# tensor4all/tensor4all-rs

Hardware: AMD Instinct MI355X
Metric: TCI2 full-sweep GF/s (d=30, chi=256 fp64) (higher is better)
Workload: dtype f64

## Files before the change

### tensor4all-rs_amd/csrc/kernels.hpp

```cpp
#pragma once

#include <hip/hip_runtime.h>

#include <cstddef>
#include <cstdint>

#include "../../include/t4a_testfunctions.h"

namespace t4a {

struct RrluWorkspace;

struct RrluPlan {
    int W = 1;
    int T = 256;
    int cpw = 0;
    int Mld = 0;
    size_t lds_bytes = 0;
};

RrluPlan rrlu_make_plan(int M, int N, int num_cus);

struct RrluArgs {
    const double* A;
// ... 90 lines not shown
    unsigned long long* trace;
    int fused;
    const uint64_t* rowacc;
    const uint64_t* colacc;
    FnDevice fn;
    unsigned done_token;
    const int* dims;
    int dims_swap;
    unsigned dev_token;
    const int* rowmap;
    int ts_u64;
};
bool rrlu_reg_make_plan(int M, int N, int num_cus, RrluRegPlan* out);
size_t rrlu_reg_keys_bytes(const RrluRegPlan& plan);
size_t rrlu_reg_cols_bytes(const RrluRegPlan& plan, int M);
void rrlu_reg_launch(const RrluRegPlan& plan, const RrluRegArgs& args, hipStream_t stream, bool keys_zeroed = false);

struct XcdSpecArgs {
    double* out;
    const uint64_t* dep_acc;
    const uint64_t* w_site;
    const uint64_t* ext_acc;
    const int* ext_cnt;
    const uint64_t* ind_acc;
    const int* ind_cnt;
    unsigned* tile_counter;
    int total, d;
    FnDevice fn;
};
struct RrluXcdPlan {
    int W = 1;
    int RPT = 1, CPT = 1;
    int grid = 8;
    size_t lds_bytes = 0;
    int wg = 0;
    int K = 1;
    bool big() const { return K > 1 || RPT > 16; }
};
struct RrluXcdArgs {
    const double* A;
    double* Aout;
    double* urows;
    int M, N;
    int max_steps;
    double rel_tol, abs_tol;
    int tie_row_major;
    int out_transposed;
    int W;
    int xcc;
    unsigned* ticket;
    unsigned ticket_base;
    int* row_perm;
    int* col_perm;
    int* iresult;
    double* dresult;
    double* pivot_vals;
    unsigned long long* keys;
    unsigned salt;
    double spec_frac;
    unsigned long long* stamps;
    unsigned long long* h_block;
    int block_u64;
    const int* dims;
    int dims_swap;
    const int* rowmap;
    XcdSpecArgs spec;
    int ts_u64;
};
bool rrlu_xcd_make_plan(int M, int N, RrluXcdPlan* out, bool any_size = false, int max_w = 32, bool allow_big = false);
size_t rrlu_xcd_keys_bytes(const RrluXcdPlan& plan);
size_t rrlu_xcd_cols_bytes(const RrluXcdPlan& plan, int M);
struct RrluXcdGroupArgs {
    RrluXcdArgs p[8];
};
void rrlu_xcd2_launch(const RrluXcdPlan& plan, const RrluXcdArgs& args, hipStream_t stream);
void rrlu_xcd2m_launch(const RrluXcdPlan& plan, const RrluXcdArgs& args, hipStream_t stream);
void rrlu_xcd2_group_launch(const RrluXcdPlan& plan, const RrluXcdGroupArgs& args, bool tie_row_major, hipStream_t stream);
bool rrlu_wg_make_plan(int M, int N, RrluXcdPlan* out, int spec_blocks = 0);
void rrlu_wg_launch(const RrluXcdPlan& plan, const RrluXcdArgs& args, hipStream_t stream);
void rrlu_wg_group_launch(const RrluXcdPlan& plan, const RrluXcdGroupArgs& args, bool tie_row_major, hipStream_t stream);
bool rrlu_w1_make_plan(int M, int N, RrluXcdPlan* out, int spec_blocks = 0);
void rrlu_w1_launch(const RrluXcdPlan& plan, const RrluXcdArgs& args, hipStream_t stream);
void rrlu_w1_group_launch(const RrluXcdPlan& plan, const RrluXcdGroupArgs& args, bool tie_row_major, hipStream_t stream);

void pi_eval_launch(const FnDevice& fn, const uint64_t* rowacc, int M, const uint64_t* colacc, int N, double* out,
                    int ld, bool transpose_out, unsigned long long* max_abs_bits, hipStream_t stream);
struct PiJob {
    const uint64_t* rowacc;
    const uint64_t* colacc;
    double* out;
    unsigned long long* max_abs_bits;
    int M, N, ld, pad_;
};
void pi_eval_batched_launch(const FnDevice& fn, const PiJob* d_jobs, int n_jobs, int max_M, int max_N, hipStream_t stream);
struct PackJob {
    const double* src;
    double* core;
    const int* info;
    int ld, L, S, R, last, pad_;
};
struct LuProblem;
constexpr int FILL_SMALL_MAX_N = 32, FILL_SMALL_MAX_RHS = 64;
void fill_small_launch(const FnDevice& fn, const PiJob* d_pis, const LuProblem* d_lups, const PackJob* d_packs, int n_jobs, int last_site,
                       hipStream_t stream);
void stage_copy_launch(const uint64_t* pinned_src, uint64_t* dst, size_t count, hipStream_t stream);
void absmax_launch(const double* data, size_t count, unsigned long long* max_abs_bits, hipStream_t stream);

constexpr int CHAIN_MAX_SET = 1024;
struct ChainTab {
    uint64_t* code;
    uint64_t* acc;
    int* cnt;
};
struct ChainCommon {
    ChainTab I, J, HI, HJ;
    ChainTab mI, mJ;
    int cap, K;
    const uint64_t* w;
    int total;
    const int* ldim;
    const int* woff;
    int forward, use_extras;
    int one_site;
    uint64_t* ind_code;
    uint64_t* ind_acc;
    int* ind_cnt;
    int ind_cap;
    uint64_t* dep_code;
    uint64_t* dep_acc;
    int dep_cap;
    int* rowmap;
    int* dims;
    int* hdims;
    uint64_t* snap_dst;
    int* snap_cnt_dst;
    size_t snap_words;
    int n_sites;
    uint64_t* zero_a;
    size_t zero_a_words;
    uint64_t* zero_b;
    size_t zero_b_words;
};
struct ChainPrepArgs {
    int b;
    int do_build;
    int with_rowmap;
    int prev_b;
    const int* prev_iresult;
    const int* prev_rowperm;
    const int* prev_colperm;
    unsigned prev_token;
    unsigned long long* dbg;
    int defer_host_writes;
};
struct ChainWalkArgs {
    char* blocks;
    size_t block_bytes, off_piv, off_rp, off_cp, off_ts;
    double* pi;
    int n_bonds;
    int max_steps;
    double rel_tol, abs_tol;
    double* factors;
    size_t factors_stride;
    unsigned token_base;
    int timed;
    int lean_prep;
    unsigned long long* phase_ticks;
};
void chain_walk_launch(const ChainCommon& c, const FnDevice& fn, const ChainWalkArgs& w, int columns, hipStream_t stream);
void chain_indep_launch(const ChainCommon& c, int n_bonds, hipStream_t stream);
void chain_last_core_launch(const ChainCommon& c, const FnDevice& fn, double* core, int max_entries, hipStream_t stream);
void chain_prep_launch(const ChainCommon& c, const ChainPrepArgs& a, hipStream_t stream);
void chain_pi_launch(const ChainCommon& c, const FnDevice& fn, int b, int n_dep_ub, int n_ind_ub, double* out, hipStream_t stream);

constexpr int CHAIN_GROUP_MAX = 8;
struct ChainGroupSlot {
    ChainCommon c;
    FnDevice fn;
    double* pi;
};
struct ChainPrepGroupArgs {
    ChainPrepArgs a[CHAIN_GROUP_MAX];
};
void chain_indep_group_launch(const ChainGroupSlot* d_slots, int n_handles, int n_bonds, hipStream_t stream);
void chain_prep_group_launch(const ChainGroupSlot* d_slots, const ChainPrepGroupArgs& a, int n_handles, hipStream_t stream);
void chain_pi_group_launch(const ChainGroupSlot* d_slots, int n_handles, int b, int n_dep_ub, int n_ind_ub, hipStream_t stream);

struct GemmDesc {
    int m, n, k;
    const double* A; int lda; long long strideA; int transA;
    const double* B; int ldb; long long strideB; int transB;
    double* C; int ldc; long long strideC;
    double alpha, beta;
    int batch;
    int ksplit = 1;
    double* partial = nullptr;
};
void gemm_launch(const GemmDesc& d, hipStream_t stream);

constexpr int LUCI_LEFT_CORES_MAX_JOBS = 80;
constexpr int LUCI_LEFT_CORES_MAX_RANK = 16;
struct LeftCoreJob {
    const double* lu;
    const int* dims;
    const int* iresult;
    const int* row_perm;
    double* core;
    int S;
    unsigned token;
};
struct LeftCoreJobs {
    LeftCoreJob j[LUCI_LEFT_CORES_MAX_JOBS];
};
void luci_left_cores_batched_launch(const LeftCoreJobs& jobs, int n_jobs, int max_rows, hipStream_t stream);
bool luci_factors_small_launch(const double* lu, int M, int N, int rk, const int* row_perm, const int* col_perm, bool left_orth,
                               double* left, double* right, hipStream_t stream);
void transpose_launch(const double* in, int rows, int cols, int ldi, double* out, int ldo, hipStream_t stream);

struct TrsmProblem {
    const double* T; int ldt; int n;
    double* B; int ldb; int nrhs;
    int lower; int unit_diag;
    const int* skip_flag;
};
void trsm_left_batched_launch(const TrsmProblem* d_problems, int n_problems, int max_n, int max_nrhs, hipStream_t stream);

struct LuProblem {
    double* A; int lda; int n;
    int* piv;
    int* info;
    double* B; int ldb; int nrhs;
    const unsigned long long* pmax_bits;
};
void lu_batched_launch(const LuProblem* d_problems, int n_problems, int max_n, hipStream_t stream);
constexpr int LU_MAX_PANEL_STEPS = 128;
bool lu_forward_blocked_launch(const LuProblem* d_problems, int n_problems, int max_n, int max_nrhs, hipStream_t stream, int avoid_xcc = -1,
                               unsigned* tickets = nullptr);
bool lu_solve_blocked_launch(const LuProblem* d_problems, int n_problems, int max_n, int max_nrhs, hipStream_t stream, int avoid_xcc = -1,
                             unsigned* tickets = nullptr);

void gather_launch(const double* in, int ldi, const int* rows, int nrows, const int* cols, int ncols, double* out,
                   int ldo, hipStream_t stream);
void scatter_rows_launch(const double* in, int ldi, const int* rows, int nrows, int ncols, double* out, int ldo,
                         hipStream_t stream);
void scatter_cols_launch(const double* in, int ldi, int nrows, const int* cols, int ncols, double* out, int ldo,
                         hipStream_t stream);
void fill_launch(double* p, size_t count, double value, hipStream_t stream);
void seq_matmul_launch(const double* A, int lda, const double* B, int ldb, double* C, int ldc, size_t M, size_t N, size_t K,
                       hipStream_t stream);
void set_identity_launch(double* p, int m, int n, int ld, hipStream_t stream);

struct TtCoreDesc { const double* data; int l, d, r; };
void tt_evaluate_launch(const TtCoreDesc* d_cores, int n_sites, int max_bond, const uint32_t* d_idx, int n_pts,
                        double* d_out, hipStream_t stream);


void core_reshape_launch(const double* in, int L, int S, int R, int mode, double* out, hipStream_t stream);
constexpr int PERMUTE_MAX_RANK = 16;
void permute_launch(const double* in, const size_t* dims, const size_t* perm, int rank, double* out, hipStream_t stream);
void tt_sum_launch(const TtCoreDesc* d_cores, int n_sites, int max_bond, double* d_out, hipStream_t stream);
void tt_norm2_step_launch(const TtCoreDesc& core, const double* d_cur, bool first, double* d_nxt, hipStream_t stream);
void tt_env_left_launch(const TtCoreDesc* d_cores, int split, int max_bond, const uint32_t* d_idx, int n_items,
                        double* d_out, int ld, hipStream_t stream);
void tt_env_right_launch(const TtCoreDesc* d_cores, int n_sites, int split, int max_bond, const uint32_t* d_idx,
                         int n_items, double* d_out, int ld, hipStream_t stream);
void tt_env_dot_launch(const double* d_left, const double* d_right, int len, int ld, const uint32_t* d_il,
                       const uint32_t* d_ir, size_t n_pts, double* d_out, hipStream_t stream);

struct MpoSiteJob {
    const double* A;
    const double* B;
    double* C;
    unsigned long long off;
    int la, s1, k, ra, lb, t, rb, pad_;
};
void mpo_site_contract_launch(const MpoSiteJob* d_jobs, int n_jobs, unsigned long long total, hipStream_t stream);

constexpr int SMALL_CAP = 16;
constexpr int SMALL_TILE = 32;
constexpr int SMALL_MAX_SITES = 32;
constexpr int SMALL_MAX_ITER = 64;
constexpr int SMALL_MAX_W = 512;
struct SmallHeader {
    int n, K, fid, total;
    int max_iter, ncheck, sweep_strategy, flags;
    int max_bond_dim, cap_in, tile_max, pad1;
    double tolerance, max_sample_value;
    double params[T4A_FN_MAX_PARAMS];
    int o_ldim, o_woff, o_w, o_cnt, o_code, o_acc, o_cores, bytes;
};
struct SmallOutHeader {
    int status;
    int iters_done;
    int converged, termination, n_pivot_errors, final_done, hist_valid, reason;
    double max_sample_value;
    unsigned long long clocks[12];
};
struct SmallOutLayout {
    size_t o_err, o_rank, o_bond, o_pe, o_shapes, o_cdims, o_cnt, o_code, o_hcnt, o_hcode, o_flag, bytes;
};
__host__ __device__ inline SmallOutLayout small_out_layout(int n)
{
    SmallOutLayout L;
    size_t o = (sizeof(SmallOutHeader) + 15) / 16 * 16;
    L.o_err = o;    o += sizeof(double) * SMALL_MAX_ITER;
    L.o_rank = o;   o += sizeof(int) * SMALL_MAX_ITER;
// ... 51 lines not shown
```

### tensor4all-rs_amd/csrc/kernels_chain.hip

```cpp
#include "kernels.hpp"
#include "kernels_rrlu_w1_body.hpp"

namespace t4a {

namespace {

__device__ __forceinline__ const char* chain_kernarg_base()
{
#if defined(__HIP_DEVICE_COMPILE__)
    return (const char*)__builtin_amdgcn_kernarg_segment_ptr();
#else
    return nullptr;
#endif
}

constexpr int CHAIN_T = 1024;
constexpr int WALK_T = 1024;
constexpr int CHAIN_HASH = 4096;

__device__ __forceinline__ unsigned chain_hash(unsigned long long c)
{
    c ^= c >> 33;
    c *= 0xff51afd7ed558ccdull;
    c ^= c >> 29;
// ... 135 lines not shown

constexpr int WALK_MAX_BONDS = 128;
constexpr int WALK_MAX_LIST = 64;
constexpr int WALK_MAX_IND = 32;
constexpr int WALK_MAX_W = 512;
struct WalkShared {
    int prev_ires[4];
    int perm_rp[WALK_MAX_LIST], perm_cp[WALK_MAX_LIST];
    int np;
    int pad_;
    uint64_t par_code[WALK_MAX_LIST], par_acc[WALK_MAX_LIST * T4A_FN_MAX_ACC];
    uint64_t dep_code[WALK_MAX_LIST], dep_acc[WALK_MAX_LIST * T4A_FN_MAX_ACC];
    int dims[WALK_MAX_BONDS * 4];
    int ind_cnt[WALK_MAX_BONDS];
    uint64_t ind_code[2][WALK_MAX_IND], ind_acc[2][WALK_MAX_IND * T4A_FN_MAX_ACC];
    uint64_t ext_code[2][WALK_MAX_LIST], ext_acc[2][WALK_MAX_LIST * T4A_FN_MAX_ACC];
    int ext_cnt[2];
    int ldim[WALK_MAX_BONDS + 1], woff[WALK_MAX_BONDS + 1];
    uint64_t w[WALK_MAX_W];
};

__device__ __forceinline__ void chain_prep_body(const ChainCommon& c, const ChainPrepArgs& p, unsigned long long* dbg = nullptr, WalkShared* ws = nullptr)
{
    unsigned long long dbg_last = dbg ? wall_clock64() : 0ull;
    auto stamp = [&](int slot) {
        if (dbg) {
            const unsigned long long now = wall_clock64();
            if (threadIdx.x == 0) dbg[slot] += now - dbg_last;
            dbg_last = now;
        }
    };
    __shared__ unsigned long long hkeys[CHAIN_HASH];
    __shared__ int wave_sums[CHAIN_T / 64];
    __shared__ int s_srcpos[CHAIN_MAX_SET];
    __shared__ int s_poison;
    const int tid = threadIdx.x;
    const int K = c.K;
    const size_t cap = (size_t)c.cap;
    if (tid == 0) s_poison = 0;
    __syncthreads();

    int n_prev_dep = 0;
    if (p.prev_b >= 0) {
        const int pb = p.prev_b;
        const int* pd = c.dims + (size_t)pb * 4;
        const int pm = pd[0], pn = pd[1];
        const bool bad = pd[2] != 0 || p.prev_iresult[1] != 0 || p.prev_iresult[3] != (int)p.prev_token || pm <= 0 || pn <= 0;
        if (bad) {
            if (tid == 0) s_poison = 1;
        } else {
            const int r = p.prev_iresult[0];
            const int cnt = r > 0 ? r : 1;
            if (cnt > c.cap || cnt > pm || cnt > pn) {
                if (tid == 0) s_poison = 1;
            } else {
                n_prev_dep = c.forward ? pm : pn;
                const uint64_t* const pind_code = ws ? ws->ind_code[pb & 1] : c.ind_code + (size_t)pb * c.ind_cap;
                const uint64_t* const pind_acc = ws ? ws->ind_acc[pb & 1] : c.ind_acc + (size_t)pb * c.ind_cap * K;
                const uint64_t* rcode = c.forward ? c.dep_code : pind_code;
                const uint64_t* racc = c.forward ? c.dep_acc : pind_acc;
                const uint64_t* ccode = c.forward ? pind_code : c.dep_code;
                const uint64_t* cacc = c.forward ? pind_acc : c.dep_acc;
                const size_t oi = (size_t)(pb + 1) * cap, oj = (size_t)pb * cap;
                for (int k = tid; k < cnt; k += (int)blockDim.x) {
                    const int ri = r > 0 ? p.prev_rowperm[k] : 0, ci = r > 0 ? p.prev_colperm[k] : 0;
                    const uint64_t rc = rcode[ri], cc = ccode[ci];
                    c.I.code[oi + k] = rc;
                    c.J.code[oj + k] = cc;
                    if (ws) ws->par_code[k] = c.forward ? rc : cc;
                    if (!p.defer_host_writes) {
                        c.mI.code[oi + k] = rc;
                        c.mJ.code[oj + k] = cc;
                    }
                    for (int q = 0; q < K; ++q) {
                        const uint64_t ra = racc[(size_t)ri * K + q], ca = cacc[(size_t)ci * K + q];
                        c.I.acc[(oi + k) * K + q] = ra;
                        c.J.acc[(oj + k) * K + q] = ca;
                        if (ws) ws->par_acc[(size_t)k * K + q] = c.forward ? ra : ca;
                        if (!p.defer_host_writes) {
                            c.mI.acc[(oi + k) * K + q] = ra;
                            c.mJ.acc[(oj + k) * K + q] = ca;
                        }
                    }
                    s_srcpos[k] = c.forward ? ri : ci;
                }
                if (tid == 0) {
                    if (ws) ws->np = cnt;
                    c.I.cnt[pb + 1] = cnt;
                    c.J.cnt[pb] = cnt;
                    if (!p.defer_host_writes) {
                        c.mI.cnt[pb + 1] = cnt;
                        c.mJ.cnt[pb] = cnt;
                    }
                }
            }
        }
        __threadfence_block();
        __syncthreads();
    }
    stamp(4);
    if (!p.do_build) return;
    const int b = p.b;
    int* dims = c.dims + (size_t)b * 4;
    int* hdims = (c.hdims && !p.defer_host_writes) ? c.hdims + (size_t)b * 4 : nullptr;
    if (s_poison) {
        if (tid == 0) {
            dims[0] = dims[1] = dims[3] = 0;
            dims[2] = 1;
            if (hdims) {
                hdims[0] = hdims[1] = 0;
                hdims[2] = 1;
            }
        }
        return;
    }

    const bool mapped = p.prev_b >= 0 && p.with_rowmap;
    int nd = -1, lda = 0;
    const bool par_lds = ws != nullptr && p.prev_b >= 0;
    const uint64_t* const xcode = ws ? ws->ext_code[b & 1] : (c.forward ? c.HI.code + (size_t)(b + 1) * cap : c.HJ.code + (size_t)b * cap);
    const uint64_t* const xacc = ws ? ws->ext_acc[b & 1] : (c.forward ? c.HI.acc + (size_t)(b + 1) * cap * K : c.HJ.acc + (size_t)b * cap * K);
    if (c.forward) {
        const int np = par_lds ? ws->np : c.I.cnt[b], ne = c.use_extras ? (ws ? ws->ext_cnt[b & 1] : c.HI.cnt[b + 1]) : 0;
        if (np >= 1 && np <= c.cap && ne <= c.cap)
            nd = build_side<true>(par_lds ? ws->par_code : c.I.code + (size_t)b * cap, par_lds ? ws->par_acc : c.I.acc + (size_t)b * cap * K, np, c.ldim[b], c.w, K, c.total, c.woff[b],
                                  xcode, xacc, ne, c.dep_code, c.dep_acc, c.dep_cap,
                                  s_srcpos, n_prev_dep, mapped ? c.rowmap : nullptr, hkeys, wave_sums);
        lda = n_prev_dep * c.ldim[b] + ne;
    } else {
        const int np = par_lds ? ws->np : c.J.cnt[b + 1], ne = c.use_extras ? (ws ? ws->ext_cnt[b & 1] : c.HJ.cnt[b]) : 0;
        if (np >= 1 && np <= c.cap && ne <= c.cap)
            nd = build_side<false>(par_lds ? ws->par_code : c.J.code + (size_t)(b + 1) * cap, par_lds ? ws->par_acc : c.J.acc + (size_t)(b + 1) * cap * K, np, c.ldim[b + 1], c.w, K, c.total,
                                   c.woff[b + 1], xcode, xacc, ne, c.dep_code, c.dep_acc,
                                   c.dep_cap, s_srcpos, n_prev_dep, mapped ? c.rowmap : nullptr, hkeys, wave_sums);
        lda = n_prev_dep * c.ldim[b + 1] + ne;
    }
    stamp(5);
    if (tid == 0) {
        const int ni = c.ind_cnt[b];
        const bool ok = nd > 0 && ni > 0;
        const int M = c.forward ? nd : ni, N = c.forward ? ni : nd;
        dims[0] = ok ? M : 0;
        dims[1] = ok ? N : 0;
        dims[2] = ok ? 0 : 1;
        dims[3] = mapped ? lda : (ok ? nd : 0);
        if (hdims) {
            hdims[0] = ok ? M : 0;
            hdims[1] = ok ? N : 0;
            hdims[2] = ok ? 0 : 1;
        }
    }
}

__global__ void __launch_bounds__(CHAIN_T) chain_prep_kernel(ChainCommon c, ChainPrepArgs p)
{
    const unsigned long long t0 = p.dbg ? wall_clock64() : 0ull;
    chain_prep_body(c, p, p.dbg);
    if (p.dbg && threadIdx.x == 0) p.dbg[6] += wall_clock64() - t0;
}
__global__ void __launch_bounds__(CHAIN_T) chain_prep_group_kernel(const ChainGroupSlot* __restrict__ slots, ChainPrepGroupArgs g)
{
    const ChainPrepArgs* pa = reinterpret_cast<const ChainPrepArgs*>(chain_kernarg_base() + sizeof(const ChainGroupSlot*)) + blockIdx.x;
    (void)g;
    chain_prep_body(slots[blockIdx.x].c, *pa);
}

__device__ __forceinline__ void chain_pi_body(const ChainCommon& c, const FnDevice& fn, int b, double* __restrict__ out)
{
    const int* dm = c.dims + (size_t)b * 4;
    if (dm[2] != 0) return;
    const int K = fn.n_acc;
    const int nd = c.forward ? dm[0] : dm[1], ni = c.forward ? dm[1] : dm[0];
    const int i = blockIdx.x * blockDim.x + threadIdx.x;
    if (blockIdx.x * (int)blockDim.x >= nd) return;
    uint64_t racc[T4A_FN_MAX_ACC] = {0, 0, 0, 0};
    if (i < nd)
        for (int k = 0; k < K; ++k) racc[k] = c.dep_acc[(size_t)i * K + k];
    const uint64_t* ia = c.ind_acc + (size_t)b * c.ind_cap * K;
    for (int j = blockIdx.y; j < ni; j += gridDim.y) {
        if (i < nd) {
            uint64_t acc[T4A_FN_MAX_ACC] = {0, 0, 0, 0};
            for (int k = 0; k < K; ++k) acc[k] = racc[k] + ia[(size_t)j * K + k];
            out[(size_t)j * nd + i] = t4a_fn_value(fn.fid, acc, fn.params);
        }
    }
}
__global__ void __launch_bounds__(256) chain_pi_kernel(ChainCommon c, FnDevice fn, int b, double* __restrict__ out) { chain_pi_body(c, fn, b, out); }
__global__ void __launch_bounds__(256) chain_pi_group_kernel(const ChainGroupSlot* __restrict__ slots, int b)
{
    const ChainGroupSlot& s = slots[blockIdx.z];
    chain_pi_body(s.c, s.fn, b, s.pi);
}


__device__ __forceinline__ void chain_mirror_body(const ChainCommon& c, int nb)
{
    const int K = c.K;
    const size_t cap = (size_t)c.cap;
    const int gtid = (int)(blockIdx.x * blockDim.x + threadIdx.x), gsz = (int)(gridDim.x * blockDim.x);
    const int lane = (int)(threadIdx.x & 63), gwave = gtid >> 6, nwaves = gsz >> 6;
    for (int pf = gwave; pf < 2 * (nb + 1); pf += nwaves) {
        const int site = pf >> 1, fam = pf & 1;
        if ((fam == 0 && site == 0) || (fam == 1 && site == nb)) continue;
        const ChainTab& T = fam == 0 ? c.I : c.J;
        const ChainTab& Mr = fam == 0 ? c.mI : c.mJ;
        const int cnt = __hip_atomic_load(T.cnt + site, __ATOMIC_RELAXED, __HIP_MEMORY_SCOPE_AGENT);
        if (cnt < 0 || cnt > c.cap) continue;
        for (int e = lane; e < cnt * (1 + K); e += 64) {
            if (e < cnt) Mr.code[(size_t)site * cap + e] = T.code[(size_t)site * cap + e];
            else Mr.acc[(size_t)site * cap * K + (e - cnt)] = T.acc[(size_t)site * cap * K + (e - cnt)];
        }
        if (lane == 0) Mr.cnt[site] = cnt;
    }
    if (c.hdims)
        for (int e = gtid; e < nb * 4; e += gsz)
            if ((e & 3) != 3) c.hdims[e] = __hip_atomic_load(c.dims + e, __ATOMIC_RELAXED, __HIP_MEMORY_SCOPE_AGENT);
}

__global__ void __launch_bounds__(256) chain_last_core_kernel(ChainCommon c, FnDevice fn, double* __restrict__ core, int max_entries)
{
    const int site = c.n_sites - 1, K = c.K;
    const size_t cap = (size_t)c.cap;
    const int L = c.I.cnt[site], R = c.J.cnt[site], S = c.ldim[site], woff = c.woff[site];
    if (L < 1 || L > c.cap || R < 1 || R > c.cap || S < 1) return;
    const long long total = (long long)L * S * R;
    if (total > (long long)max_entries) return;
    for (long long e = (long long)blockIdx.x * blockDim.x + threadIdx.x; e < total; e += (long long)gridDim.x * blockDim.x) {
        const int l = (int)(e % L), s_ = (int)((e / L) % S), r = (int)(e / ((long long)L * S));
        uint64_t acc[T4A_FN_MAX_ACC] = {0, 0, 0, 0};
        for (int q = 0; q < K; ++q)
            acc[q] = c.I.acc[((size_t)site * cap + l) * K + q] + c.w[(size_t)q * c.total + woff + s_] + c.J.acc[((size_t)site * cap + r) * K + q];
        core[e] = t4a_fn_value(fn.fid, acc, fn.params);
    }
}

__device__ __forceinline__ void walk_phase_barrier(bool scalar_cache = true)
{
    if (scalar_cache) {
        __syncthreads();
        __builtin_amdgcn_s_dcache_inv();
        asm volatile("s_waitcnt lgkmcnt(0)" ::: "memory");
    } else {
        asm volatile("s_waitcnt lgkmcnt(0)\n\ts_barrier" ::: "memory");
    }
}
__device__ __forceinline__ int walk_div_small(int x, float rd) { return (int)(((float)x + 0.5f) * rd); }
__device__ __forceinline__ int walk_load_i32(const int* p) { return __hip_atomic_load(p, __ATOMIC_RELAXED, __HIP_MEMORY_SCOPE_AGENT); }

template <bool FORWARD>
__device__ __forceinline__ void walk_prep_wave0(const ChainCommon& c, WalkShared* ws, int b, int prev_b, unsigned prev_token, bool do_build, unsigned long long* dbg = nullptr)
{
    const unsigned long long dbg_t0 = dbg ? wall_clock64() : 0ull;
    const int lane = threadIdx.x & 63;
    const int K = c.K;
    const size_t cap = (size_t)c.cap;
    bool poison = false;
    int np = 0;
    if (prev_b >= 0) {
        const int pb = prev_b;
        const int pm = ws->dims[pb * 4], pn = ws->dims[pb * 4 + 1];
        const bool bad = ws->dims[pb * 4 + 2] != 0 || ws->prev_ires[1] != 0 || ws->prev_ires[3] != (int)prev_token || pm <= 0 || pn <= 0;
        const int r = ws->prev_ires[0];
        const int cnt = r > 0 ? r : 1;
        if (bad || cnt > c.cap || cnt > pm || cnt > pn || cnt > WALK_MAX_LIST) {
            poison = true;
        } else {
            const uint64_t* const pind_code = ws->ind_code[pb & 1];
            const uint64_t* const pind_acc = ws->ind_acc[pb & 1];
            uint64_t rc = 0, cc = 0, ra[T4A_FN_MAX_ACC] = {0, 0, 0, 0}, ca[T4A_FN_MAX_ACC] = {0, 0, 0, 0};
            if (lane < cnt) {
                const int ri = r > 0 ? ws->perm_rp[lane] : 0, ci = r > 0 ? ws->perm_cp[lane] : 0;
                rc = FORWARD ? ws->dep_code[ri] : pind_code[ri];
                cc = FORWARD ? pind_code[ci] : ws->dep_code[ci];
                for (int q = 0; q < K; ++q) {
                    ra[q] = FORWARD ? ws->dep_acc[(size_t)ri * K + q] : pind_acc[(size_t)ri * K + q];
                    ca[q] = FORWARD ? pind_acc[(size_t)ci * K + q] : ws->dep_acc[(size_t)ci * K + q];
                }
            }
            if (lane < cnt) {
                const size_t oi = (size_t)(pb + 1) * cap, oj = (size_t)pb * cap;
                c.I.code[oi + lane] = rc;
                c.J.code[oj + lane] = cc;
                ws->par_code[lane] = FORWARD ? rc : cc;
                for (int q = 0; q < K; ++q) {
                    c.I.acc[(oi + lane) * K + q] = ra[q];
                    c.J.acc[(oj + lane) * K + q] = ca[q];
                    ws->par_acc[(size_t)lane * K + q] = FORWARD ? ra[q] : ca[q];
                }
            }
            if (lane == 0) {
                c.I.cnt[pb + 1] = cnt;
                c.J.cnt[pb] = cnt;
            }
            np = cnt;
        }
    }
    const unsigned long long dbg_t1 = dbg ? wall_clock64() : 0ull;
    if (dbg && (threadIdx.x & 63) == 0) dbg[4] += dbg_t1 - dbg_t0;
    if (!do_build) return;
    int* const dims = ws->dims + b * 4;
    if (poison) {
        if (lane == 0) {
            dims[0] = dims[1] = dims[3] = 0;
            dims[2] = 1;
        }
        return;
    }
    const int site = FORWARD ? b : b + 1;
    const int d = c.ldim[site], woff = c.woff[site];
    const ChainTab& PT = FORWARD ? c.I : c.J;
// ... 314 lines not shown
```

### tensor4all-rs_amd/csrc/tci2_chain.hip

```cpp
#include "tci2.hpp"

#include <algorithm>
#include <atomic>
#include <chrono>
#include <cmath>
#include <cstdlib>

namespace t4a {

namespace {
size_t round_up_sz(size_t v, size_t m) { return (v + m - 1) / m * m; }
std::atomic<int> g_chains_inflight{0};
}
thread_local double g_chain_wait_seconds = 0.0;

bool Tci2::chain_usable(const TCI2Options& options) const
{
    static const bool off = std::getenv("T4A_NO_CHAIN") != nullptr;
    if (off || !chain_enabled || fn_kind_ != FnKind::Builtin || options.pivot_search != 0) return false;
    long double space = 1.0L;
    for (size_t d : local_dims) space *= (long double)d;
    if (space >= 9.0e18L) return false;
    for (size_t p = 0; p < n_; ++p) {
        if (i_set[p].count == 0 || j_set[p].count == 0) return false;
// ... 328 lines not shown
        }
    }
    int snap = -1;
    if (in_optimize) {
        snap = use_extras ? 1 - ext_slot : 0;
        chain_.snap_serial[snap] = chain_.hist_serial;
    }

    for (size_t b = 0; b < nb; ++b) {
        std::memset(chain_.hblocks.get() + b * proto.bytes, 0, 32);
        std::memset(chain_.hdims.get() + b * 4, 0xFF, 4 * sizeof(int));
    }
    ChainCommon c;
    std::memset(&c, 0, sizeof(c));
    c.I = chain_tab(0);
    c.J = chain_tab(1);
    c.HI = chain_tab(2 + 2 * ext_slot);
    c.HJ = chain_tab(3 + 2 * ext_slot);
    c.mI = chain_mirror(1 - chain_.mcur, 0);
    c.mJ = chain_mirror(1 - chain_.mcur, 1);
    c.cap = (int)cap;
    c.K = (int)K;
    c.w = chain_.weights.get();
    c.total = (int)total_;
    c.ldim = chain_.siteinfo.get();
    c.woff = chain_.siteinfo.get() + n_;
    c.forward = forward ? 1 : 0;
    c.use_extras = use_extras ? 1 : 0;
    c.one_site = one ? 1 : 0;
    c.ind_code = chain_.ind.get();
    c.ind_acc = chain_.ind.get() + nb * ind_cap;
    c.ind_cnt = chain_.ind_cnt.get();
    c.ind_cap = (int)ind_cap;
    c.dep_code = chain_.dep.get();
    c.dep_acc = chain_.dep.get() + dep_cap;
    c.dep_cap = (int)dep_cap;
    c.rowmap = chain_.rowmap.get();
    c.dims = chain_.dims.get();
    c.hdims = chain_.hdims.get();
    c.n_sites = (int)n_;
    if (snap >= 0) {
        c.snap_dst = chain_tab(2 + 2 * snap).code;
        c.snap_cnt_dst = chain_tab(2 + 2 * snap).cnt;
        c.snap_words = 2 * n_ * cap * (1 + K);
    }
    c.zero_a = reinterpret_cast<uint64_t*>(chain_.blocks.get());
    c.zero_a_words = nb * proto.bytes / 8;
    c.zero_b = reinterpret_cast<uint64_t*>(chain_.dims.get());
    c.zero_b_words = (nb * 5 * sizeof(int) + 7) / 8;

    chain_.common = c;
    chain_.prepared = true;
    chain_.forward = forward;
    chain_.in_optimize = in_optimize;
    chain_.ext_idx = ext_idx;
    chain_.chi = chi;
    chain_.tol = options.tolerance;
    chain_.order = std::move(order);
    chain_.plans = std::move(plans);
    chain_.dep_ub = std::move(dep_ub);
    chain_.ind_ub = std::move(ind_ub);
    chain_.use_extras = use_extras;
    chain_.ind_cap = ind_cap;
    chain_.cap_side = cap_side;
    chain_.proto = proto;
    chain_.timed = timed;
    chain_.timed_events = timed_events;
    chain_.tokens.assign(nb, 0u);
    if (launch) chain_launch();
    return true;
}

void Tci2::chain_launch()
{
    if (!chain_.prepared) throw Error(T4A_GPU_INTERNAL_ERROR, "bond chain: nothing prepared to launch");
    chain_.prepared = false;
    const size_t nb = n_ - 1;
    const size_t K = (size_t)chain_.n_acc, cap = chain_.cap;
    const bool forward = chain_.forward, use_extras = chain_.use_extras, timed_events = chain_.timed_events;
    const size_t chi = chain_.chi, ind_cap = chain_.ind_cap, cap_side = chain_.cap_side;
    const ChainCommon& c = chain_.common;
    const RrluBlock& proto = chain_.proto;
    const std::vector<size_t>& order = chain_.order;
    const std::vector<RrluRoute>& plans = chain_.plans;
    const std::vector<size_t>& dep_ub = chain_.dep_ub;
    const std::vector<size_t>& ind_ub = chain_.ind_ub;
    std::vector<unsigned>& tokens = chain_.tokens;
    hipStream_t st = eng.stream();
    auto block_of = [&](size_t b) {
        RrluBlock k = proto;
        k.dev = chain_.blocks.get() + b * proto.bytes;
        return k;
    };
    {
        size_t reserve_words = 0;
        const RrluRoute cr = cap_side ? eng.chain_route((int)cap_side, (int)cap_side) : RrluRoute();
        if (cr.on_xcd()) reserve_words = cr.xcd_mailbox_words();
        eng.chain_begin(plans, reserve_words);
    }
    bool counted = false;
    try {
        chain_indep_launch(c, (int)nb, st);
        unsigned* tile_counters = reinterpret_cast<unsigned*>(chain_.dims.get() + nb * 4);
        const bool solo = g_chains_inflight.fetch_add(1) == 0;
        counted = true;
        static const bool no_walk = std::getenv("T4A_NO_WALK") != nullptr;
        size_t walk_cols = 0;
        bool walk = !no_walk && !timed_events && nb <= 128;
        for (size_t b = 0; walk && b < nb; ++b) {
            walk = dep_ub[b] <= 64 && ind_ub[b] <= 32;
            walk_cols = std::max(walk_cols, ind_ub[b]);
        }
        if (walk) {
            ChainWalkArgs w;
            std::memset(&w, 0, sizeof(w));
            w.blocks = chain_.blocks.get();
            w.block_bytes = proto.bytes;
            w.off_piv = proto.off_piv;
            w.off_rp = proto.off_rp;
            w.off_cp = proto.off_cp;
            w.off_ts = proto.off_ts;
            w.pi = chain_.pi.get();
            w.n_bonds = (int)nb;
            w.max_steps = (int)std::min<size_t>(chi, 64);
            w.rel_tol = chain_.tol;
            w.abs_tol = chain_.one_site ? chain_.abs_tol : 0.0;
            w.factors = chain_.factors_stride ? chain_.factors.get() : nullptr;
            w.factors_stride = chain_.factors_stride;
            if (chain_.walk_token > 0xFFFF0000u || chain_.walk_token == 0u) chain_.walk_token = 1u;
            w.token_base = chain_.walk_token;
            chain_.walk_token += (unsigned)nb;
            w.timed = chain_.timed ? 1 : 0;
            w.lean_prep = 1;
            static const bool walk_dbg = std::getenv("T4A_WALK_DEBUG") != nullptr;
            if (walk_dbg) {
                chain_.walk_dbg.reserve(8);
                T4A_HIP(hipMemsetAsync(chain_.walk_dbg.get(), 0, 8 * sizeof(unsigned long long), st));
                w.phase_ticks = chain_.walk_dbg.get();
            }
            chain_.walked = true;
            for (size_t k = 0; k < nb; ++k) tokens[order[k]] = w.token_base + (unsigned)k;
            chain_walk_launch(c, fn_dev_, w, (int)walk_cols, st);
            ++chain_stats_ext[0];
        }
        static const bool want_prep_dbg = std::getenv("T4A_PREP_DEBUG") != nullptr;
        unsigned long long* prep_dbg = nullptr;
        if (want_prep_dbg && !walk) {
            chain_.walk_dbg.reserve(8);
            T4A_HIP(hipMemsetAsync(chain_.walk_dbg.get(), 0, 8 * sizeof(unsigned long long), st));
            prep_dbg = chain_.walk_dbg.get();
            chain_.prep_dbg = true;
        }
        bool spec_pending = false;
        for (size_t k = 0; !walk && k < nb; ++k) {
            const size_t b = order[k];
            const RrluRoute& pl = plans[b];
            const bool fused = pl.fused;
            const bool spec_here = spec_pending && !fused;
            const RrluBlock blk = block_of(b);
            ChainPrepArgs pa;
            std::memset(&pa, 0, sizeof(pa));
            pa.b = (int)b;
            pa.do_build = 1;
            pa.dbg = prep_dbg;
            pa.defer_host_writes = 0;
            pa.with_rowmap = spec_here ? 1 : 0;
            pa.prev_b = -1;
            if (k > 0) {
                const size_t pb = order[k - 1];
                const RrluBlock pblk = block_of(pb);
                pa.prev_b = (int)pb;
                pa.prev_iresult = pblk.iresult();
                pa.prev_rowperm = pblk.row_perm();
                pa.prev_colperm = pblk.col_perm();
                pa.prev_token = tokens[pb];
            }
            chain_prep_launch(c, pa, st);
            if (!fused && !spec_here) chain_pi_launch(c, fn_dev_, (int)b, (int)dep_ub[b], (int)ind_ub[b], chain_.pi.get(), st);
            XcdSpecArgs sp;
            std::memset(&sp, 0, sizeof(sp));
            spec_pending = false;
            if (solo && k + 1 < nb && pl.on_xcd()) {
                const size_t nx = order[k + 1];
                if (!plans[nx].fused) {
                    const size_t site = forward ? nx : nx + 1;
                    const ChainTab& H = forward ? c.HI : c.HJ;
                    const size_t hsite = forward ? nx + 1 : nx;
                    sp.out = chain_.spec[(k + 1) & 1].get();
                    sp.dep_acc = c.dep_acc;
                    sp.w_site = c.w + offset_[site];
                    sp.ext_acc = H.acc + hsite * cap * K;
                    sp.ext_cnt = use_extras ? H.cnt + hsite : nullptr;
                    sp.ind_acc = c.ind_acc + nx * ind_cap * K;
                    sp.ind_cnt = c.ind_cnt + nx;
                    sp.tile_counter = tile_counters + nx;
                    sp.total = (int)total_;
                    sp.d = (int)local_dims[site];
                    sp.fn = fn_dev_;
                    spec_pending = true;
                }
            }
            FusedPi fp;
            fp.fn = fn_dev_;
            fp.d_rowacc = c.dep_acc;
            fp.d_colacc = c.ind_acc + b * ind_cap * K;
            fp.host_resident = false;
            const double* A = fused ? nullptr : (spec_here ? chain_.spec[k & 1].get() : chain_.pi.get());
            if (timed_events) T4A_HIP(hipEventRecord(chain_.t0[b], st));
            tokens[b] = eng.chain_rrlu(pl, forward, A, spec_here ? c.rowmap : nullptr, fused ? &fp : nullptr, c.dims + b * 4, chi, chain_.tol,
                                       chain_.one_site ? chain_.abs_tol : 0.0, blk, spec_pending ? &sp : nullptr,
                                       chain_.factors_stride ? chain_.factors.get() + b * chain_.factors_stride : nullptr, chain_.urows.get());
            if (timed_events) T4A_HIP(hipEventRecord(chain_.t1[b], st));
        }
        if (!walk) {
            const size_t pb = order[nb - 1];
            const RrluBlock pblk = block_of(pb);
            ChainPrepArgs pa;
            std::memset(&pa, 0, sizeof(pa));
            pa.do_build = 0;
            pa.defer_host_writes = 0;
            pa.prev_b = (int)pb;
            pa.prev_iresult = pblk.iresult();
            pa.prev_rowperm = pblk.row_perm();
            pa.prev_colperm = pblk.col_perm();
            pa.prev_token = tokens[pb];
            chain_prep_launch(c, pa, st);
        }
        chain_.cores_batched = false;
        if (chain_.one_site && chain_.factors_stride && forward && nb <= (size_t)LUCI_LEFT_CORES_MAX_JOBS) {
            LeftCoreJobs jobs;
            std::memset(&jobs, 0, sizeof(jobs));
            size_t max_rows = 1;
            for (size_t b = 0; b < nb; ++b) {
                const RrluBlock blk = block_of(b);
                const size_t rub = std::max<size_t>(std::min({dep_ub[b], ind_ub[b], chi}), 1);
                DevCore& core = cores[b];
                core.buf.reserve(std::max<size_t>(dep_ub[b] * rub, 1));
                LeftCoreJob& j = jobs.j[b];
                j.lu = chain_.factors.get() + b * chain_.factors_stride;
                j.dims = c.dims + b * 4;
                j.iresult = blk.iresult();
                j.row_perm = blk.row_perm();
                j.core = core.buf.get();
                j.S = (int)local_dims[b];
                j.token = tokens[b];
                max_rows = std::max(max_rows, dep_ub[b]);
            }
            luci_left_cores_batched_launch(jobs, (int)nb, (int)max_rows, st);
            chain_.cores_batched = true;
        }
        chain_.last_core_launched = false;
        if (chain_.one_site && chain_.factors_stride && forward) {
            const size_t last = n_ - 1;
            const size_t a_ub = std::max<size_t>(std::min({dep_ub[nb - 1], ind_ub[nb - 1], chi}), 1);
            const size_t entries = a_ub * local_dims[last] * std::max<size_t>(j_set[last].count, 1);
            if (entries <= ((size_t)1 << 24)) {
                cores[last].buf.reserve(entries);
                chain_last_core_launch(c, fn_dev_, cores[last].buf.get(), (int)entries, st);
                chain_.last_core_launched = true;
            }
        }
        T4A_HIP(hipMemcpyAsync(chain_.hblocks.get(), chain_.blocks.get(), nb * proto.bytes, hipMemcpyDeviceToHost, st));
        T4A_HIP(hipGetLastError());
    } catch (...) {
        (void)hipStreamSynchronize(st);
        eng.chain_end();
        if (counted) g_chains_inflight.fetch_sub(1);
        chain_.tables_valid = false;
        chain_.snap_serial[0] = chain_.snap_serial[1] = ~0ull;
        throw;
    }
    chain_.inflight = true;
    chain_.wait_stream = st;
    chain_.group_role = 0;
}

void Tci2::chain_group_launch(const std::vector<Tci2*>& hs)
{
    const size_t nh = hs.size();
    if (nh == 0) return;
    bool ok = nh >= 2 && nh <= (size_t)CHAIN_GROUP_MAX;
    Tci2* lead = hs[0];
    for (Tci2* h : hs) {
        if (!h->chain_.prepared) throw Error(T4A_GPU_INTERNAL_ERROR, "bond chain: a handle of the group has nothing prepared");
        ok = ok && h->n_ == lead->n_ && h->chain_.forward == lead->chain_.forward && h->chain_.chi == lead->chain_.chi &&
             h->chain_.tol == lead->chain_.tol && !h->chain_.timed_events;
    }
    const size_t nb = lead->n_ - 1;
    const bool forward = lead->chain_.forward;
    std::vector<RrluRoute> gplans(nb);
    size_t side_ub = 0;
    if (ok) {
        for (size_t b = 0; b < nb && ok; ++b) {
            size_t dm = 1, im = 1;
            for (Tci2* h : hs) {
                dm = std::max(dm, h->chain_.dep_ub[b]);
                im = std::max(im, h->chain_.ind_ub[b]);
            }
            gplans[b] = Engine::chain_group_route((int)dm, (int)im);
            ok = gplans[b].ok();
        }
        for (Tci2* h : hs) side_ub = std::max(side_ub, h->chain_.cap_side);
    }
    if (!ok) {
        for (Tci2* h : hs) h->chain_launch();
        return;
    }
    hipStream_t st = lead->eng.stream();
    size_t reserve_words = 0;
    {
        const RrluRoute cr = side_ub ? Engine::chain_group_route((int)side_ub, (int)side_ub) : RrluRoute();
        if (cr.ok()) reserve_words = cr.xcd_mailbox_words();
    }
    std::vector<char> counted(nh, 0);
    bool locked = false;
    try {
        lead->chain_.gslots.reserve(CHAIN_GROUP_MAX);
        lead->chain_.hgslots.reserve(CHAIN_GROUP_MAX);
        for (size_t i = 0; i < nh; ++i) {
            Tci2* h = hs[i];
            h->chain_.prepared = false;
            if (h != lead) {
                if (!h->chain_.group_ev) T4A_HIP(hipEventCreateWithFlags(&h->chain_.group_ev, hipEventDisableTiming));
                T4A_HIP(hipEventRecord(h->chain_.group_ev, h->eng.stream()));
                T4A_HIP(hipStreamWaitEvent(st, h->chain_.group_ev, 0));
            }
            h->eng.chain_group_reserve(gplans, reserve_words, st);
            ChainGroupSlot& slot = lead->chain_.hgslots.get()[i];
            slot.c = h->chain_.common;
            slot.fn = h->fn_dev_;
            slot.pi = h->chain_.pi.get();
            g_chains_inflight.fetch_add(1);
            counted[i] = 1;
        }
        T4A_HIP(hipMemcpyAsync(lead->chain_.gslots.get(), lead->chain_.hgslots.get(), nh * sizeof(ChainGroupSlot), hipMemcpyHostToDevice, st));
        const ChainGroupSlot* d_slots = lead->chain_.gslots.get();
        lead->eng.chain_group_lock();
        locked = true;
        auto block_of = [&](Tci2* h, size_t b) {
            RrluBlock k = h->chain_.proto;
            k.dev = h->chain_.blocks.get() + b * k.bytes;
            return k;
        };
        auto prev_of = [&](Tci2* h, size_t pb, ChainPrepArgs& pa) {
            const RrluBlock pblk = block_of(h, pb);
            pa.prev_b = (int)pb;
            pa.prev_iresult = pblk.iresult();
            pa.prev_rowperm = pblk.row_perm();
            pa.prev_colperm = pblk.col_perm();
            pa.prev_token = h->chain_.tokens[pb];
        };
        chain_indep_group_launch(d_slots, (int)nh, (int)nb, st);
        const std::vector<size_t>& order = lead->chain_.order;
        for (size_t k = 0; k < nb; ++k) {
            const size_t b = order[k];
            ChainPrepGroupArgs pg;
            std::memset(&pg, 0, sizeof(pg));
            for (size_t i = 0; i < nh; ++i) {
                ChainPrepArgs& pa = pg.a[i];
                pa.b = (int)b;
                pa.do_build = 1;
                pa.prev_b = -1;
                if (k > 0) prev_of(hs[i], order[k - 1], pa);
            }
            chain_prep_group_launch(d_slots, pg, (int)nh, st);
            chain_pi_group_launch(d_slots, (int)nh, (int)b, gplans[b].kM, gplans[b].kN, st);
            RrluXcdGroupArgs ga;
            std::memset(&ga, 0, sizeof(ga));
            for (int x = 0; x < 8; ++x) ga.p[x].xcc = -1;
            for (size_t i = 0; i < nh; ++i) {
                Tci2* h = hs[i];
                h->chain_.tokens[b] = h->eng.chain_group_args(gplans[b], forward, h->chain_.pi.get(), h->chain_.common.dims + b * 4, h->chain_.chi,
                                                              h->chain_.tol, 0.0, block_of(h, b), (int)i, &ga.p[i], st);
            }
            gplans[b].launch_group(ga, !forward, st);
        }
        {
            ChainPrepGroupArgs pg;
// ... 294 lines not shown
```

Baseline: 304.1.

## Add latency-optimized chain prep kernel with front-loaded loads and LDS hashing

Replaces the chain prep kernel body with a new variant that issues every independent global load up front (previous dims, iresult, row/column permutations, table entries, extras, gathered accumulators) before a single barrier. It also stages the weight slice in LDS and compacts the kept extras with a ballot and per-wave sums. A permutation length is passed from the host so the permutation loads can be speculated before the poison check. The goal is to cut the serialized dependent-latency chain in a small, latency-bound per-bond kernel. It adds more LDS use and duplicates the logic, which carries a risk of divergence from the original body. The group kernel still uses the old body.

```diff
diff --git a/tensor4all-rs_amd/csrc/kernels.hpp b/tensor4all-rs_amd/csrc/kernels.hpp
--- a/tensor4all-rs_amd/csrc/kernels.hpp
+++ b/tensor4all-rs_amd/csrc/kernels.hpp
@@ -266,6 +266,7 @@
     unsigned prev_token;
     unsigned long long* dbg;
     int defer_host_writes;
+    int prev_perm_len;
 };
 struct ChainWalkArgs {
     char* blocks;
diff --git a/tensor4all-rs_amd/csrc/kernels_chain.hip b/tensor4all-rs_amd/csrc/kernels_chain.hip
--- a/tensor4all-rs_amd/csrc/kernels_chain.hip
+++ b/tensor4all-rs_amd/csrc/kernels_chain.hip
@@ -311,10 +311,249 @@
     }
 }
 
+constexpr int PREP_W_MAX = 1024;
+
+__device__ __forceinline__ void prep_lds_barrier() { asm volatile("s_waitcnt lgkmcnt(0)\n\ts_barrier" ::: "memory"); }
+
+__device__ __forceinline__ void chain_prep_fast_body(const ChainCommon& c, const ChainPrepArgs& p, unsigned long long* dbg)
+{
+    static_assert(CHAIN_MAX_SET <= CHAIN_T, "chain_prep_fast_body: one thread per table entry");
+    unsigned long long dbg_last = dbg ? wall_clock64() : 0ull;
+    auto stamp = [&](int slot) {
+        if (dbg) {
+            const unsigned long long now = wall_clock64();
+            if (threadIdx.x == 0) dbg[slot] += now - dbg_last;
+            dbg_last = now;
+        }
+    };
+    __shared__ unsigned long long hkeys[CHAIN_HASH];
+    __shared__ uint64_t s_w[PREP_W_MAX];
+    __shared__ int wave_sums[CHAIN_T / 64];
+    const int tid = threadIdx.x, lane = tid & 63, wave = tid >> 6;
+    const int K = c.K, cap = c.cap;
+    const bool fw = c.forward != 0;
+    const bool gather = p.prev_b >= 0, build = p.do_build != 0;
+    const int b = p.b, pb = p.prev_b;
+    const int site = fw ? b : b + 1;
+    const int hsite = fw ? b + 1 : b;
+    const ChainTab& T = fw ? c.I : c.J;
+    const ChainTab& H = fw ? c.HI : c.HJ;
+
+    int pm = 0, pn = 0, pbad = 0, r = 0, ir1 = 0, ir3 = 0, srp = 0, scp = 0;
+    if (gather) {
+        const int* pd = c.dims + (size_t)pb * 4;
+        pm = pd[0];
+        pn = pd[1];
+        pbad = pd[2];
+        r = p.prev_iresult[0];
+        ir1 = p.prev_iresult[1];
+        ir3 = p.prev_iresult[3];
+        if (tid < p.prev_perm_len) {
+            srp = p.prev_rowperm[tid];
+            scp = p.prev_colperm[tid];
+        }
+    }
+    int ni = 0, d = 1, wo = 0, ne = 0, np_tab = 0;
+    uint64_t ec = 0ull, tc = 0ull;
+    uint64_t ea[T4A_FN_MAX_ACC], ta[T4A_FN_MAX_ACC];
+    if (build) {
+        ni = c.ind_cnt[b];
+        d = c.ldim[site];
+        wo = c.woff[site];
+        if (!gather) {
+            np_tab = T.cnt[site];
+            if (tid < cap) {
+                tc = T.code[(size_t)site * cap + tid];
+#pragma unroll
+                for (int q = 0; q < T4A_FN_MAX_ACC; ++q)
+                    if (q < K) ta[q] = T.acc[((size_t)site * cap + tid) * K + q];
+            }
+        }
+        if (c.use_extras) {
+            ne = H.cnt[hsite];
+            if (tid < cap) {
+                ec = H.code[(size_t)hsite * cap + tid];
+#pragma unroll
+                for (int q = 0; q < T4A_FN_MAX_ACC; ++q)
+                    if (q < K) ea[q] = H.acc[((size_t)hsite * cap + tid) * K + q];
+            }
+            for (int e = tid; e < CHAIN_HASH; e += (int)blockDim.x) hkeys[e] = 0ull;
+        }
+    }
+
+    bool poison = false;
+    int cnt = 0;
+    if (gather) {
+        poison = pbad != 0 || ir1 != 0 || ir3 != (int)p.prev_token || pm <= 0 || pn <= 0;
+        cnt = r > 0 ? r : 1;
+        if (!poison && (cnt > cap || cnt > pm || cnt > pn)) poison = true;
+    }
+    const int n_prev_dep = gather && !poison ? (fw ? pm : pn) : 0;
+
+    const bool gathers = gather && !poison && tid < cnt;
+    int ri = 0, ci = 0;
+    uint64_t rc = 0ull, cc = 0ull;
+    uint64_t ra[T4A_FN_MAX_ACC], ca[T4A_FN_MAX_ACC];
+    if (gathers) {
+        ri = r > 0 ? (tid < p.prev_perm_len ? srp : p.prev_rowperm[tid]) : 0;
+        ci = r > 0 ? (tid < p.prev_perm_len ? scp : p.prev_colperm[tid]) : 0;
+        const uint64_t* const pind_code = c.ind_code + (size_t)pb * c.ind_cap;
+        const uint64_t* const pind_acc = c.ind_acc + (size_t)pb * c.ind_cap * K;
+        const uint64_t* rcode = fw ? c.dep_code : pind_code;
+        const uint64_t* racc = fw ? c.dep_acc : pind_acc;
+        const uint64_t* ccode = fw ? pind_code : c.dep_code;
+        const uint64_t* cacc = fw ? pind_acc : c.dep_acc;
+        rc = rcode[ri];
+        cc = ccode[ci];
+#pragma unroll
+        for (int q = 0; q < T4A_FN_MAX_ACC; ++q)
+            if (q < K) {
+                ra[q] = racc[(size_t)ri * K + q];
+                ca[q] = cacc[(size_t)ci * K + q];
+            }
+    }
+    const bool w_lds = K * d <= PREP_W_MAX;
+    if (build && !poison && w_lds)
+        for (int t = tid; t < K * d; t += (int)blockDim.x) s_w[t] = c.w[(size_t)(t / d) * c.total + wo + t % d];
+    asm volatile("s_waitcnt vmcnt(0) lgkmcnt(0)\n\ts_barrier" ::: "memory");
+
+    if (gathers) {
+        const size_t oi = (size_t)(pb + 1) * cap + tid, oj = (size_t)pb * cap + tid;
+        if (!p.defer_host_writes) {
+            c.mI.code[oi] = rc;
+            c.mJ.code[oj] = cc;
+#pragma unroll
+            for (int q = 0; q < T4A_FN_MAX_ACC; ++q)
+                if (q < K) {
+                    c.mI.acc[oi * K + q] = ra[q];
+                    c.mJ.acc[oj * K + q] = ca[q];
+                }
+        }
+        c.I.code[oi] = rc;
+        c.J.code[oj] = cc;
+#pragma unroll
+        for (int q = 0; q < T4A_FN_MAX_ACC; ++q)
+            if (q < K) {
+                c.I.acc[oi * K + q] = ra[q];
+                c.J.acc[oj * K + q] = ca[q];
+            }
+        if (tid == 0) {
+            if (!p.defer_host_writes) {
+                c.mI.cnt[pb + 1] = cnt;
+                c.mJ.cnt[pb] = cnt;
+            }
+            c.I.cnt[pb + 1] = cnt;
+            c.J.cnt[pb] = cnt;
+        }
+    }
+    stamp(4);
+    if (!build) return;
+    int* dims = c.dims + (size_t)b * 4;
+    int* hdims = (c.hdims && !p.defer_host_writes) ? c.hdims + (size_t)b * 4 : nullptr;
+    if (poison) {
+        if (tid == 0) {
+            dims[0] = dims[1] = dims[3] = 0;
+            dims[2] = 1;
+            if (hdims) {
+                hdims[0] = hdims[1] = 0;
+                hdims[2] = 1;
+            }
+        }
+        return;
+    }
+
+    const bool mapped = gather && p.with_rowmap;
+    const int np = gather ? cnt : np_tab;
+    const int lda = n_prev_dep * d + ne;
+    const int m0 = np * d;
+    int nd = -1;
+    if (np >= 1 && np <= cap && ne <= cap && m0 <= c.dep_cap) {
+        if (tid < np) {
+            const uint64_t pc = gather ? (fw ? rc : cc) : tc;
+            const int src = fw ? ri : ci;
+            for (int s = 0; s < d; ++s) {
+                const int idx = fw ? tid * d + s : s * np + tid;
+                c.dep_code[idx] = (uint64_t)s + (uint64_t)d * pc;
+#pragma unroll
+                for (int q = 0; q < T4A_FN_MAX_ACC; ++q)
+                    if (q < K) {
+                        const uint64_t pa = gather ? (fw ? ra[q] : ca[q]) : ta[q];
+                        const uint64_t wv = w_lds ? s_w[q * d + s] : c.w[(size_t)q * c.total + wo + s];
+                        c.dep_acc[(size_t)idx * K + q] = pa + wv;
+                    }
+                if (mapped) c.rowmap[idx] = src * d + s;
+            }
+            if (ne > 0) {
+                const unsigned long long key = (unsigned long long)pc + 1ull;
+                unsigned h = chain_hash(key);
+                for (;;) {
+                    const unsigned long long old = atomicCAS(&hkeys[h], 0ull, key);
+                    if (old == 0ull || old == key) break;
+                    h = (h + 1) & (CHAIN_HASH - 1);
+                }
+            }
+        }
+        if (ne <= 0) {
+            nd = m0;
+        } else {
+            prep_lds_barrier();
+            bool keep = false;
+            if (tid < ne) {
+                const unsigned long long key = (unsigned long long)(ec / (uint64_t)d) + 1ull;
+                unsigned h = chain_hash(key);
+                keep = true;
+                for (;;) {
+                    const unsigned long long v = hkeys[h];
+                    if (v == 0ull) break;
+                    if (v == key) {
+                        keep = false;
+                        break;
+                    }
+                    h = (h + 1) & (CHAIN_HASH - 1);
+                }
+            }
+            const unsigned long long bal = __ballot(keep);
+            if (lane == 0) wave_sums[wave] = __builtin_popcountll(bal);
+            prep_lds_barrier();
+            int base = 0, tot = 0;
+            for (int w = 0; w < (int)blockDim.x / 64; ++w) {
+                const int v = wave_sums[w];
+                if (w < wave) base += v;
+                tot += v;
+            }
+            if (m0 + tot <= c.dep_cap) {
+                if (keep) {
+                    const int o = m0 + base + __builtin_popcountll(bal & ((1ull << lane) - 1ull));
+                    c.dep_code[o] = ec;
+#pragma unroll
+                    for (int q = 0; q < T4A_FN_MAX_ACC; ++q)
+                        if (q < K) c.dep_acc[(size_t)o * K + q] = ea[q];
+                    if (mapped) c.rowmap[o] = n_prev_dep * d + tid;
+                }
+                nd = m0 + tot;
+            }
+        }
+    }
+    stamp(5);
+    if (tid == 0) {
+        const bool ok = nd > 0 && ni > 0;
+        const int M = fw ? nd : ni, N = fw ? ni : nd;
+        dims[0] = ok ? M : 0;
+        dims[1] = ok ? N : 0;
+        dims[2] = ok ? 0 : 1;
+        dims[3] = mapped ? lda : (ok ? nd : 0);
+        if (hdims) {
+            hdims[0] = ok ? M : 0;
+            hdims[1] = ok ? N : 0;
+            hdims[2] = ok ? 0 : 1;
+        }
+    }
+}
+
 __global__ void __launch_bounds__(CHAIN_T) chain_prep_kernel(ChainCommon c, ChainPrepArgs p)
 {
     const unsigned long long t0 = p.dbg ? wall_clock64() : 0ull;
-    chain_prep_body(c, p, p.dbg);
+    chain_prep_fast_body(c, p, p.dbg);
     if (p.dbg && threadIdx.x == 0) p.dbg[6] += wall_clock64() - t0;
 }
 __global__ void __launch_bounds__(CHAIN_T) chain_prep_group_kernel(const ChainGroupSlot* __restrict__ slots, ChainPrepGroupArgs g)
diff --git a/tensor4all-rs_amd/csrc/tci2_chain.hip b/tensor4all-rs_amd/csrc/tci2_chain.hip
--- a/tensor4all-rs_amd/csrc/tci2_chain.hip
+++ b/tensor4all-rs_amd/csrc/tci2_chain.hip
@@ -504,6 +504,7 @@
             chain_.prep_dbg = true;
         }
         bool spec_pending = false;
+        const int perm_len = (int)std::min((proto.off_cp - proto.off_rp) / sizeof(int), (proto.off_ts - proto.off_cp) / sizeof(int));
         for (size_t k = 0; !walk && k < nb; ++k) {
             const size_t b = order[k];
             const RrluRoute& pl = plans[b];
@@ -526,6 +527,7 @@
                 pa.prev_rowperm = pblk.row_perm();
                 pa.prev_colperm = pblk.col_perm();
                 pa.prev_token = tokens[pb];
+                pa.prev_perm_len = perm_len;
             }
             chain_prep_launch(c, pa, st);
             if (!fused && !spec_here) chain_pi_launch(c, fn_dev_, (int)b, (int)dep_ub[b], (int)ind_ub[b], chain_.pi.get(), st);
@@ -576,6 +578,7 @@
             pa.prev_rowperm = pblk.row_perm();
             pa.prev_colperm = pblk.col_perm();
             pa.prev_token = tokens[pb];
+            pa.prev_perm_len = perm_len;
             chain_prep_launch(c, pa, st);
         }
         chain_.cores_batched = false;
```

Result: no change. 304.5 (median of 6 runs) (+0.1%).
